# ViktorLiang/GW-Depth

Hardware: AMD Instinct MI355X
Metric: images/sec (train fwd+bwd) 480x640 bs=8/GPU (higher is better)
Workload: dtype bf16; 1 GPU; GW-Depth full model (res50 + DETR 6+6 + 4-scale ReferTransformer + decoder) fwd+17 losses+bwd+clip+AdamW, 480x640, bs=8/GPU, dropout 0.1; global_batch=8, parallelism=dp1, launch=hipgraph, graph_segments=1, grad_buckets=8

## Files before the change

gw_depth_amd/csrc/pyrtail.hip:

```cpp
#include "common.h"

namespace {

constexpr int PT_TH = 8, PT_TW = 8;
constexpr int PT_CH = 32;
constexpr int PT_MAXCHUNK = 10;
constexpr int PT_MAXR = 5, PT_MAXC = 5;
constexpr int PT_MAXPOS = PT_MAXR * PT_MAXC;
constexpr int PT_TAB = 128;
constexpr int PT_SPLIT = 4;

struct PyrBranches {
    void *p[GWD_PYR_MAX_BRANCHES];
    int h[GWD_PYR_MAX_BRANCHES], w[GWD_PYR_MAX_BRANCHES];
    int start[GWD_PYR_MAX_BRANCHES + 1];
    int n;
};

__device__ __forceinline__ float pt_scale(int in, int out) { return out > 1 ? (float)(in - 1) / (float)(out - 1) : 0.f; }

__device__ __forceinline__ float pt_weight(int o, int s, int in, float scale) {
    const float f = scale * o;
    const int i0 = (int)f, i1 = i0 + (i0 < in - 1);
    const float l = f - i0;
    return (i0 == s ? 1.f - l : 0.f) + (i1 == s ? l : 0.f);
}

template <typename T> struct Vec8;
template <> struct alignas(16) Vec8<__bf16> { __bf16 e[8]; };
template <> struct alignas(16) Vec8<float> { float e[8]; };

template <typename T> struct Raw8;
template <> struct Raw8<__bf16> { uint4 a; };
template <> struct Raw8<float> { uint4 a, b; };

template <typename T>
__device__ __forceinline__ void fma8(float (&acc)[8], float wgt, const Vec8<T> &v) {
#pragma unroll
    for (int e = 0; e < 8; ++e) acc[e] = fmaf(wgt, to_f32(v.e[e]), acc[e]);
}

template <typename T>
__global__ __launch_bounds__(256) void pyr_tail_fwd_kernel(const T *__restrict__ part, const PyrBranches br, const float *__restrict__ gamma,
                                                           const float *__restrict__ beta, T *__restrict__ z, T *__restrict__ y,
                                                           float *__restrict__ mean, float *__restrict__ rstd, int H, int W, int N, int gelu) {
    __shared__ Vec8<T> smz[PT_MAXPOS * 36];
    __shared__ Vec8<float> smh[PT_MAXR * 3 * PT_TW * 4];
    const int t = threadIdx.x, q = t & 3, pix = t >> 2;
    const int ntx = (W + PT_TW - 1) / PT_TW, nty = (H + PT_TH - 1) / PT_TH;
    const long vb = xcd_grouped_block(blockIdx.x, gridDim.x, 2 * ntx);
    const int px0 = (int)(vb % ntx) * PT_TW, py0 = (int)((vb / ntx) % nty) * PT_TH, b = (int)(vb / ((long)ntx * nty));
    const int pxl = pix & (PT_TW - 1);
    const int px = px0 + pxl, py = py0 + pix / PT_TW;
    const bool inside = px < W && py < H;
    const int nch = N / PT_CH;
    float acc[PT_MAXCHUNK][8];
#pragma unroll
    for (int j = 0; j < PT_MAXCHUNK; ++j)
#pragma unroll
        for (int e = 0; e < 8; ++e) acc[j][e] = 0.f;
    const int ya = max(py0 - 1, 0), yb = min(py0 + PT_TH, H - 1), xa = max(px0 - 1, 0), xb = min(px0 + PT_TW, W - 1);
    for (int k = 0; k < br.n; ++k) {
        const int h = br.h[k], w = br.w[k];
        const float sh = pt_scale(h, H), sw = pt_scale(w, W);
        const int rlo = (int)(sh * ya), rhi = min((int)(sh * yb) + 1, h - 1);
        const int clo = (int)(sw * xa), chi = min((int)(sw * xb) + 1, w - 1);
        const int nc = min(chi - clo + 1, PT_MAXC), nr = min(rhi - rlo + 1, PT_MAXR);
        const T *Zk = (const T *)br.p[k] + (size_t)b * h * w * 9 * N;
        static_assert(PT_MAXPOS * 36 <= 4 * 256, "four window places a thread");
        const int nitem = nr * nc * 36;
        auto place = [&](int u) {
            const int i = min(t + u * 256, nitem - 1);
            const int pos = i / 36, rem = i - pos * 36;
            return (((rlo + pos / nc) * w + clo + pos % nc) * 9 + (rem >> 2)) * N + (rem & 3) * 8;
        };
        const int zoff0 = place(0), zoff1 = place(1), zoff2 = place(2), zoff3 = place(3);
        typedef Raw8<T> R8;
        R8 pre0 = *(const R8 *)(Zk + zoff0), pre1 = *(const R8 *)(Zk + zoff1), pre2 = *(const R8 *)(Zk + zoff2), pre3 = *(const R8 *)(Zk + zoff3);
        R8 *smr = (R8 *)smz;
#pragma unroll
        for (int j = 0; j < PT_MAXCHUNK; ++j) {
            if (j < nch) {
                if (t < nitem) smr[t] = pre0;
                if (t + 256 < nitem) smr[t + 256] = pre1;
                if (t + 512 < nitem) smr[t + 512] = pre2;
                if (t + 768 < nitem) smr[t + 768] = pre3;
                __syncthreads();
                if (j + 1 < nch) {
                    const T *Zn = Zk + (j + 1) * PT_CH;
                    pre0 = *(const R8 *)(Zn + zoff0);
                    pre1 = *(const R8 *)(Zn + zoff1);
                    pre2 = *(const R8 *)(Zn + zoff2);
                    pre3 = *(const R8 *)(Zn + zoff3);
                }
                for (int i = t; i < nr * 3 * PT_TW * 4; i += 256) {
                    const int lane = i & 3, xl = (i >> 2) & (PT_TW - 1), rt = i / (PT_TW * 4);
                    const int rr = rt / 3, ty = rt - rr * 3;
                    Vec8<float> hv;
#pragma unroll
                    for (int e = 0; e < 8; ++e) hv.e[e] = 0.f;
#pragma unroll
                    for (int tx = 0; tx < 3; ++tx) {
                        const int xx = px0 + xl + tx - 1;
                        if (xx < 0 || xx >= W) continue;
                        const float fx = sw * xx;
                        const int c0 = (int)fx, c1 = c0 + (c0 < w - 1);
                        const float lx = fx - c0, hx = 1.f - lx;
                        const int tq = (ty * 3 + tx) * 4 + lane;
                        fma8<T>(hv.e, hx, smz[(rr * nc + min(c0 - clo, PT_MAXC - 1)) * 36 + tq]);
                        fma8<T>(hv.e, lx, smz[(rr * nc + min(c1 - clo, PT_MAXC - 1)) * 36 + tq]);
                    }
                    smh[i] = hv;
                }
                __syncthreads();
                if (inside) {
#pragma unroll
                    for (int ty = 0; ty < 3; ++ty) {
                        const int yy = py + ty - 1;
                        if (yy < 0 || yy >= H) continue;
                        const float fy = sh * yy;
                        const int r0 = (int)fy, r1 = r0 + (r0 < h - 1);
                        const float ly = fy - r0, hy = 1.f - ly;
                        fma8<float>(acc[j], hy, smh[((min(r0 - rlo, PT_MAXR - 1) * 3 + ty) * PT_TW + pxl) * 4 + q]);
                        fma8<float>(acc[j], ly, smh[((min(r1 - rlo, PT_MAXR - 1) * 3 + ty) * PT_TW + pxl) * 4 + q]);
                    }
                }
            }
        }
    }
    const size_t row = ((size_t)b * H + (inside ? py : 0)) * W + (inside ? px : 0);
    float s = 0.f;
#pragma unroll
    for (int j = 0; j < PT_MAXCHUNK; ++j) {
        if (j < nch && inside) {
            const size_t off = row * N + j * PT_CH + q * 8;
            const Vec8<T> pv = *(const Vec8<T> *)(part + off);
            Vec8<T> zv;
#pragma unroll
            for (int e = 0; e < 8; ++e) {
                zv.e[e] = from_f32<T>(acc[j][e] + to_f32(pv.e[e]));
                acc[j][e] = to_f32(zv.e[e]);
                s += acc[j][e];
            }
            if (z) *(Vec8<T> *)(z + off) = zv;
        }
    }
    s += __shfl_xor(s, 1, 64);
    s += __shfl_xor(s, 2, 64);
    const float mu = s / (float)N;
    float v2 = 0.f;
#pragma unroll
    for (int j = 0; j < PT_MAXCHUNK; ++j) {
        if (j < nch) {
#pragma unroll
            for (int e = 0; e < 8; ++e) {
                const float d = acc[j][e] - mu;
                v2 += d * d;
            }
        }
    }
    v2 += __shfl_xor(v2, 1, 64);
    v2 += __shfl_xor(v2, 2, 64);
    const float rs = rsqrtf(v2 / (float)N + 1e-5f);
    if (!inside) return;
    if (q == 0) {
        mean[row] = mu;
        rstd[row] = rs;
    }
#pragma unroll
    for (int j = 0; j < PT_MAXCHUNK; ++j) {
        if (j < nch) {
            const int ch = j * PT_CH + q * 8;
            Vec8<T> ov;
#pragma unroll
            for (int e = 0; e < 8; ++e) {
                float o = (acc[j][e] - mu) * rs * gamma[ch + e] + beta[ch + e];
                if (gelu) o = gelu_t<T>(o);
                ov.e[e] = from_f32<T>(o);
            }
            *(Vec8<T> *)(y + row * N + ch) = ov;
        }
    }
}

template <typename T>
__global__ __launch_bounds__(256) void pyr_tail_bwd_kernel(const T *__restrict__ gz, const PyrBranches br, int H, int W, int N) {
    __shared__ float sm[(PT_SPLIT - 1) * 9 * (PT_MAXCHUNK * 4) * 8];
    __shared__ float tabx[PT_TAB * 3], taby[PT_TAB * 3];
    const int lanes = N / 8, lane = threadIdx.x % lanes, grp = threadIdx.x / lanes;
    int k = 0;
    while (k + 1 < br.n && (int)blockIdx.x >= br.start[k + 1]) ++k;
    const int h = br.h[k], w = br.w[k];
    const int local = (int)xcd_grouped_block(blockIdx.x - br.start[k], br.start[k + 1] - br.start[k], 2 * w);
    const int c = local % w, r = (local / w) % h, b = local / (w * h);
    const float sh = pt_scale(h, H), sw = pt_scale(w, W);
    int ylo = 0, yhi = H - 1, xlo = 0, xhi = W - 1;
    if (sh > 0.f) {
        ylo = max(0, (int)floorf((r - 1) / sh) - 2);
        yhi = min(H - 1, (int)ceilf((r + 1) / sh) + 2);
    }
    if (sw > 0.f) {
        xlo = max(0, (int)floorf((c - 1) / sw) - 2);
        xhi = min(W - 1, (int)ceilf((c + 1) / sw) + 2);
    }
    auto wx_of = [&](int xx, int tx) {
        const int sx = xx + tx - 1;
        return (sx >= 0 && sx < W) ? pt_weight(sx, c, w, sw) : 0.f;
    };
    while (xlo < xhi && wx_of(xlo, 0) == 0.f && wx_of(xlo, 1) == 0.f && wx_of(xlo, 2) == 0.f) ++xlo;
    while (xhi > xlo && wx_of(xhi, 0) == 0.f && wx_of(xhi, 1) == 0.f && wx_of(xhi, 2) == 0.f) --xhi;
    auto wy_of = [&](int yy, int ty) {
        const int sy = yy + ty - 1;
        return (sy >= 0 && sy < H) ? pt_weight(sy, r, h, sh) : 0.f;
    };
    const bool tab = xhi - xlo < PT_TAB && yhi - ylo < PT_TAB;
    if (tab) {
        for (int i = threadIdx.x; i < (xhi - xlo + 1) * 3; i += blockDim.x) tabx[i] = wx_of(xlo + i / 3, i % 3);
        for (int i = threadIdx.x; i < (yhi - ylo + 1) * 3; i += blockDim.x) taby[i] = wy_of(ylo + i / 3, i % 3);
        __syncthreads();
    }
    float acc[9][8];
#pragma unroll
    for (int i = 0; i < 9; ++i)
#pragma unroll
        for (int e = 0; e < 8; ++e) acc[i][e] = 0.f;
    const T *gb = gz + (size_t)b * H * W * N + lane * 8;
    for (int yy = ylo + grp; yy <= yhi; yy += PT_SPLIT) {
        float wy[3];
#pragma unroll
        for (int ty = 0; ty < 3; ++ty) wy[ty] = tab ? taby[(yy - ylo) * 3 + ty] : wy_of(yy, ty);
        if (wy[0] == 0.f && wy[1] == 0.f && wy[2] == 0.f) continue;
        float rowsum[3][8];
#pragma unroll
        for (int i = 0; i < 3; ++i)
#pragma unroll
            for (int e = 0; e < 8; ++e) rowsum[i][e] = 0.f;
#pragma unroll 4
        for (int xx = xlo; xx <= xhi; ++xx) {
            float wx[3];
#pragma unroll
            for (int tx = 0; tx < 3; ++tx) wx[tx] = tab ? tabx[(xx - xlo) * 3 + tx] : wx_of(xx, tx);
            const Vec8<T> v = *(const Vec8<T> *)(gb + ((size_t)yy * W + xx) * N);
#pragma unroll
            for (int tx = 0; tx < 3; ++tx) fma8<T>(rowsum[tx], wx[tx], v);
        }
#pragma unroll
        for (int ty = 0; ty < 3; ++ty)
#pragma unroll
            for (int tx = 0; tx < 3; ++tx)
#pragma unroll
                for (int e = 0; e < 8; ++e) acc[ty * 3 + tx][e] = fmaf(wy[ty], rowsum[tx][e], acc[ty * 3 + tx][e]);
    }
    if (grp > 0) {
#pragma unroll
        for (int i = 0; i < 9; ++i)
#pragma unroll
            for (int e = 0; e < 8; ++e) sm[(((grp - 1) * 9 + i) * lanes + lane) * 8 + e] = acc[i][e];
    }
    __syncthreads();
    if (grp == 0) {
        T *G = (T *)br.p[k] + ((size_t)(b * h + r) * w + c) * 9 * N + lane * 8;
#pragma unroll
        for (int i = 0; i < 9; ++i) {
            Vec8<T> ov;
#pragma unroll
            for (int e = 0; e < 8; ++e) {
                float v = acc[i][e];
#pragma unroll
                for (int g = 0; g < PT_SPLIT - 1; ++g) v += sm[((g * 9 + i) * lanes + lane) * 8 + e];
                ov.e[e] = from_f32<T>(v);
            }
            *(Vec8<T> *)(G + (size_t)i * N) = ov;
        }
    }
}

struct PyrFold {
    const float *lo[GWD_PYR_MAX_BRANCHES];
};
__global__ __launch_bounds__(256) void pyr_tail_fold_kernel(const float *__restrict__ d_hi, const PyrFold lo, float *__restrict__ dw, int N,
                                                            int C2, int nbr, int nlow, int64_t total) {
    const int64_t i = (int64_t)blockIdx.x * 256 + threadIdx.x;
    if (i >= total) return;
    const int Cw = (1 + nbr) * C2, Chi = (1 + nbr - nlow) * C2;
    const int ch = (int)(i % Cw);
    const int64_t nt = i / Cw;
    const int tap = (int)(nt % 9), n = (int)(nt / 9);
    const int g = ch / C2, ci = ch - g * C2;
    float v;
    if (g == 0) v = d_hi[nt * Chi + ci];
    else if (g <= nlow) v = lo.lo[g - 1][((size_t)tap * N + n) * C2 + ci];
    else v = d_hi[nt * Chi + (g - nlow) * C2 + ci];
    dw[i] += v;
}

int check_branches(const int32_t *hk, const int32_t *wk, int nb, int H, int W) {
    for (int k = 0; k < nb; ++k) {
        if (hk[k] <= 0 || wk[k] <= 0 || hk[k] > H || wk[k] > W) return -1;
    }
    return 0;
}

}

extern "C" int gwd_pyr_tail_forward(const void *part, const void *const *Z, const int32_t *hk, const int32_t *wk, int32_t nb,
                                    const float *gamma, const float *beta, void *z, void *y, float *mean, float *rstd, int32_t B,
                                    int32_t H, int32_t W, int32_t N, int32_t gelu, int32_t dtype, void *stream) {
    if (!part || !Z || !hk || !wk || !gamma || !beta || !y || !mean || !rstd || B <= 0 || H <= 0 || W <= 0 || N <= 0) return -1;
    if (nb < 1 || nb > GWD_PYR_MAX_BRANCHES || check_branches(hk, wk, nb, H, W)) return -1;
    if (dtype != GWD_BF16 && dtype != GWD_F32) return -2;
    if (N % PT_CH || N > PT_CH * PT_MAXCHUNK) return -4;
    PyrBranches br = {};
    br.n = nb;
    for (int k = 0; k < nb; ++k) {
        if (!Z[k]) return -1;
        const double sh = H > 1 ? (double)(hk[k] - 1) / (H - 1) : 0.0, sw = W > 1 ? (double)(wk[k] - 1) / (W - 1) : 0.0;
        int nr = (int)(sh * (PT_TH + 1) * (1.0 + 1e-6)) + 3, nc = (int)(sw * (PT_TW + 1) * (1.0 + 1e-6)) + 3;
        nr = nr < hk[k] ? nr : hk[k];
        nc = nc < wk[k] ? nc : wk[k];
        if (nr > PT_MAXR || nc > PT_MAXC) return -4;
        br.p[k] = const_cast<void *>(Z[k]);
        br.h[k] = hk[k];
        br.w[k] = wk[k];
    }
    const int64_t nblk = (int64_t)B * ((W + PT_TW - 1) / PT_TW) * ((H + PT_TH - 1) / PT_TH);
    if (nblk >= (1LL << 31)) return -7;
    const int grid = (int)nblk;
    if (dtype == GWD_BF16)
        pyr_tail_fwd_kernel<__bf16><<<grid, 256, 0, (hipStream_t)stream>>>((const __bf16 *)part, br, gamma, beta, (__bf16 *)z, (__bf16 *)y, mean,
                                                                           rstd, H, W, N, gelu);
    else
        pyr_tail_fwd_kernel<float><<<grid, 256, 0, (hipStream_t)stream>>>((const float *)part, br, gamma, beta, (float *)z, (float *)y, mean, rstd,
                                                                          H, W, N, gelu);
    GWD_CHECK_LAUNCH();
    return 0;
}

extern "C" int gwd_pyr_tail_backward(const void *gz, void *const *G, const int32_t *hk, const int32_t *wk, int32_t nb, int32_t B, int32_t H,
                                     int32_t W, int32_t N, int32_t dtype, void *stream) {
    if (!gz || !G || !hk || !wk || B <= 0 || H <= 0 || W <= 0 || N <= 0) return -1;
    if (nb < 1 || nb > GWD_PYR_MAX_BRANCHES || check_branches(hk, wk, nb, H, W)) return -1;
    if (dtype != GWD_BF16 && dtype != GWD_F32) return -2;
    if (N % 8 || N > PT_CH * PT_MAXCHUNK) return -4;
    PyrBranches br = {};
    br.n = nb;
    int64_t blocks = 0;
    for (int k = 0; k < nb; ++k) {
        if (!G[k]) return -1;
        br.p[k] = G[k];
        br.h[k] = hk[k];
        br.w[k] = wk[k];
        br.start[k] = (int)blocks;
        blocks += (int64_t)B * hk[k] * wk[k];
        if (blocks >= (1LL << 31)) return -7;
    }
    br.start[nb] = (int)blocks;
    const int threads = N / 8 * PT_SPLIT;
    if (dtype == GWD_BF16) pyr_tail_bwd_kernel<__bf16><<<(int)blocks, threads, 0, (hipStream_t)stream>>>((const __bf16 *)gz, br, H, W, N);
    else pyr_tail_bwd_kernel<float><<<(int)blocks, threads, 0, (hipStream_t)stream>>>((const float *)gz, br, H, W, N);
    GWD_CHECK_LAUNCH();
    return 0;
}

extern "C" int gwd_pyr_tail_fold_wgrad(const float *d_hi, const float *const *d_low, int32_t nlow, float *dw, int32_t N, int32_t C2,
                                       int32_t nbr, void *stream) {
    if (!d_hi || !d_low || !dw || N <= 0 || C2 <= 0 || nbr < 1 || nbr > GWD_PYR_MAX_BRANCHES || nlow < 1 || nlow > nbr) return -1;
    PyrFold lo = {};
    for (int k = 0; k < nlow; ++k) {
        if (!d_low[k]) return -1;
        lo.lo[k] = d_low[k];
    }
    const int64_t total = (int64_t)N * 9 * (1 + nbr) * C2;
    if ((total + 255) / 256 >= (1LL << 31)) return -7;
    pyr_tail_fold_kernel<<<(int)((total + 255) / 256), 256, 0, (hipStream_t)stream>>>(d_hi, lo, dw, N, C2, nbr, nlow, total);
    GWD_CHECK_LAUNCH();
    return 0;
}
```

Baseline: 264.5 images/s.

## Double-buffer pyramid tail forward, widen to 8 lanes per pixel, precompute interp offsets

The pyramid-tail forward kernel goes from 256 to 512 threads, with 8 lanes per pixel each handling 4 channels instead of 4 lanes handling 8. Window tiles and horizontal sums are double-buffered in shared memory, so the next chunk's global loads and shared stores overlap compute and one barrier per chunk is dropped. Bilinear indices and weights are hoisted out of the chunk loop into per-thread registers, and gamma and beta are loaded as float4. In the backward kernel the table/no-table branch is hoisted out of the inner loop and pointer increments replace index arithmetic. The costs are doubled shared memory and a larger block, which may lower occupancy.

```diff
diff --git a/gw_depth_amd/csrc/pyrtail.hip b/gw_depth_amd/csrc/pyrtail.hip
--- a/gw_depth_amd/csrc/pyrtail.hip
+++ b/gw_depth_amd/csrc/pyrtail.hip
@@ -3,6 +3,8 @@
 namespace {
 
 constexpr int PT_TH = 8, PT_TW = 8;
+constexpr int PT_LANES = 8;
+constexpr int PT_FTHREADS = PT_TH * PT_TW * PT_LANES;
 constexpr int PT_CH = 32;
 constexpr int PT_MAXCHUNK = 10;
 constexpr int PT_MAXR = 5, PT_MAXC = 5;
@@ -19,12 +21,24 @@
 
 __device__ __forceinline__ float pt_scale(int in, int out) { return out > 1 ? (float)(in - 1) / (float)(out - 1) : 0.f; }
 
+__device__ __forceinline__ void pt_coord(int o, float scale, int &i0, float &l) {
+#pragma clang fp contract(off)
+    const float f = scale * o;
+    i0 = (int)f;
+    l = f - i0;
+}
+
 __device__ __forceinline__ float pt_weight(int o, int s, int in, float scale) {
-    const float f = scale * o;
-    const int i0 = (int)f, i1 = i0 + (i0 < in - 1);
-    const float l = f - i0;
+    int i0;
+    float l;
+    pt_coord(o, scale, i0, l);
+    const int i1 = i0 + (i0 < in - 1);
     return (i0 == s ? 1.f - l : 0.f) + (i1 == s ? l : 0.f);
 }
+
+template <typename T> struct Vec4;
+template <> struct alignas(8) Vec4<__bf16> { __bf16 e[4]; };
+template <> struct alignas(16) Vec4<float> { float e[4]; };
 
 template <typename T> struct Vec8;
 template <> struct alignas(16) Vec8<__bf16> { __bf16 e[8]; };
@@ -35,18 +49,25 @@
 template <> struct Raw8<float> { uint4 a, b; };
 
 template <typename T>
+__device__ __forceinline__ void fma4(float (&acc)[4], float wgt, const Vec4<T> &v) {
+#pragma unroll
+    for (int e = 0; e < 4; ++e) acc[e] = fmaf(wgt, to_f32(v.e[e]), acc[e]);
+}
+
+template <typename T>
 __device__ __forceinline__ void fma8(float (&acc)[8], float wgt, const Vec8<T> &v) {
 #pragma unroll
     for (int e = 0; e < 8; ++e) acc[e] = fmaf(wgt, to_f32(v.e[e]), acc[e]);
 }
 
 template <typename T>
-__global__ __launch_bounds__(256) void pyr_tail_fwd_kernel(const T *__restrict__ part, const PyrBranches br, const float *__restrict__ gamma,
-                                                           const float *__restrict__ beta, T *__restrict__ z, T *__restrict__ y,
-                                                           float *__restrict__ mean, float *__restrict__ rstd, int H, int W, int N, int gelu) {
-    __shared__ Vec8<T> smz[PT_MAXPOS * 36];
-    __shared__ Vec8<float> smh[PT_MAXR * 3 * PT_TW * 4];
-    const int t = threadIdx.x, q = t & 3, pix = t >> 2;
+__global__ __launch_bounds__(PT_FTHREADS) __attribute__((amdgpu_waves_per_eu(2, 4))) void pyr_tail_fwd_kernel(
+    const T *__restrict__ part, const PyrBranches br, const float *__restrict__ gamma, const float *__restrict__ beta, T *__restrict__ z,
+    T *__restrict__ y, float *__restrict__ mean, float *__restrict__ rstd, int H, int W, int N, int gelu) {
+    typedef Raw8<T> R8;
+    __shared__ R8 smz[2][PT_MAXPOS * 36];
+    __shared__ Vec4<float> smh[2][PT_MAXR * 3 * PT_TW * PT_LANES];
+    const int t = threadIdx.x, q = t & (PT_LANES - 1), pix = t / PT_LANES;
     const int ntx = (W + PT_TW - 1) / PT_TW, nty = (H + PT_TH - 1) / PT_TH;
     const long vb = xcd_grouped_block(blockIdx.x, gridDim.x, 2 * ntx);
     const int px0 = (int)(vb % ntx) * PT_TW, py0 = (int)((vb / ntx) % nty) * PT_TH, b = (int)(vb / ((long)ntx * nty));
@@ -54,12 +75,13 @@
     const int px = px0 + pxl, py = py0 + pix / PT_TW;
     const bool inside = px < W && py < H;
     const int nch = N / PT_CH;
-    float acc[PT_MAXCHUNK][8];
+    float acc[PT_MAXCHUNK][4];
 #pragma unroll
     for (int j = 0; j < PT_MAXCHUNK; ++j)
 #pragma unroll
-        for (int e = 0; e < 8; ++e) acc[j][e] = 0.f;
+        for (int e = 0; e < 4; ++e) acc[j][e] = 0.f;
     const int ya = max(py0 - 1, 0), yb = min(py0 + PT_TH, H - 1), xa = max(px0 - 1, 0), xb = min(px0 + PT_TW, W - 1);
+    const Vec4<T> *smz4 = (const Vec4<T> *)smz;
     for (int k = 0; k < br.n; ++k) {
         const int h = br.h[k], w = br.w[k];
         const float sh = pt_scale(h, H), sw = pt_scale(w, W);
@@ -67,63 +89,95 @@
         const int clo = (int)(sw * xa), chi = min((int)(sw * xb) + 1, w - 1);
         const int nc = min(chi - clo + 1, PT_MAXC), nr = min(rhi - rlo + 1, PT_MAXR);
         const T *Zk = (const T *)br.p[k] + (size_t)b * h * w * 9 * N;
-        static_assert(PT_MAXPOS * 36 <= 4 * 256, "four window places a thread");
+        static_assert(PT_MAXPOS * 36 <= 2 * PT_FTHREADS, "two window places a thread");
         const int nitem = nr * nc * 36;
         auto place = [&](int u) {
-            const int i = min(t + u * 256, nitem - 1);
+            const int i = min(t + u * PT_FTHREADS, nitem - 1);
             const int pos = i / 36, rem = i - pos * 36;
             return (((rlo + pos / nc) * w + clo + pos % nc) * 9 + (rem >> 2)) * N + (rem & 3) * 8;
         };
-        const int zoff0 = place(0), zoff1 = place(1), zoff2 = place(2), zoff3 = place(3);
-        typedef Raw8<T> R8;
-        R8 pre0 = *(const R8 *)(Zk + zoff0), pre1 = *(const R8 *)(Zk + zoff1), pre2 = *(const R8 *)(Zk + zoff2), pre3 = *(const R8 *)(Zk + zoff3);
-        R8 *smr = (R8 *)smz;
+        const int zoff0 = place(0), zoff1 = place(1);
+        R8 pre0 = *(const R8 *)(Zk + zoff0), pre1 = *(const R8 *)(Zk + zoff1);
+        static_assert(PT_MAXR * 3 <= 2 * (PT_FTHREADS / 64), "two horizontal items a thread");
+        int hoff0[3], hoff1[3];
+        float hx[3], lx[3];
+#pragma unroll
+        for (int tx = 0; tx < 3; ++tx) {
+            const int xx = px0 + pxl + tx - 1;
+            const bool ok = xx >= 0 && xx < W;
+            int c0;
+            float l;
+            pt_coord(ok ? xx : 0, sw, c0, l);
+            const int c1 = c0 + (c0 < w - 1);
+            hx[tx] = ok ? 1.f - l : 0.f;
+            lx[tx] = ok ? l : 0.f;
+            hoff0[tx] = min(max(c0 - clo, 0), nc - 1) * 72 + tx * 8;
+            hoff1[tx] = min(max(c1 - clo, 0), nc - 1) * 72 + tx * 8;
+        }
+        const int rt0 = t >> 6, rt1 = rt0 + PT_FTHREADS / 64;
+        const int hbase0 = (rt0 / 3) * nc * 72 + (rt0 % 3) * 24 + q, hbase1 = (rt1 / 3) * nc * 72 + (rt1 % 3) * 24 + q;
+        const bool hdo0 = rt0 < nr * 3, hdo1 = rt1 < nr * 3;
+        int voff0[3], voff1[3];
+        float hy[3], ly[3];
+#pragma unroll
+        for (int ty = 0; ty < 3; ++ty) {
+            const int yy = py + ty - 1;
+            const bool ok = inside && yy >= 0 && yy < H;
+            int r0;
+            float l;
+            pt_coord(ok ? yy : 0, sh, r0, l);
+            const int r1 = r0 + (r0 < h - 1);
+            hy[ty] = ok ? 1.f - l : 0.f;
+            ly[ty] = ok ? l : 0.f;
+            voff0[ty] = ((min(max(r0 - rlo, 0), nr - 1) * 3 + ty) * PT_TW + pxl) * PT_LANES + q;
+            voff1[ty] = ((min(max(r1 - rlo, 0), nr - 1) * 3 + ty) * PT_TW + pxl) * PT_LANES + q;
+        }
+        if (t < nitem) smz[0][t] = pre0;
+        if (t + PT_FTHREADS < nitem) smz[0][t + PT_FTHREADS] = pre1;
+        if (nch > 1) {
+            pre0 = *(const R8 *)(Zk + PT_CH + zoff0);
+            pre1 = *(const R8 *)(Zk + PT_CH + zoff1);
+        }
+        __syncthreads();
 #pragma unroll
         for (int j = 0; j < PT_MAXCHUNK; ++j) {
             if (j < nch) {
-                if (t < nitem) smr[t] = pre0;
-                if (t + 256 < nitem) smr[t + 256] = pre1;
-                if (t + 512 < nitem) smr[t + 512] = pre2;
-                if (t + 768 < nitem) smr[t + 768] = pre3;
-                __syncthreads();
+                constexpr int PIECES = PT_MAXPOS * 72, SUMS = PT_MAXR * 3 * PT_TW * PT_LANES;
+                const Vec4<T> *wz = smz4 + (j & 1) * PIECES;
+                Vec4<float> *wh = smh[j & 1];
                 if (j + 1 < nch) {
-                    const T *Zn = Zk + (j + 1) * PT_CH;
-                    pre0 = *(const R8 *)(Zn + zoff0);
-                    pre1 = *(const R8 *)(Zn + zoff1);
-                    pre2 = *(const R8 *)(Zn + zoff2);
-                    pre3 = *(const R8 *)(Zn + zoff3);
+                    if (t < nitem) smz[(j + 1) & 1][t] = pre0;
+                    if (t + PT_FTHREADS < nitem) smz[(j + 1) & 1][t + PT_FTHREADS] = pre1;
+                    if (j + 2 < nch) {
+                        const T *Zn = Zk + (j + 2) * PT_CH;
+                        pre0 = *(const R8 *)(Zn + zoff0);
+                        pre1 = *(const R8 *)(Zn + zoff1);
+                    }
                 }
-                for (int i = t; i < nr * 3 * PT_TW * 4; i += 256) {
-                    const int lane = i & 3, xl = (i >> 2) & (PT_TW - 1), rt = i / (PT_TW * 4);
-                    const int rr = rt / 3, ty = rt - rr * 3;
-                    Vec8<float> hv;
-#pragma unroll
-                    for (int e = 0; e < 8; ++e) hv.e[e] = 0.f;
+                if (hdo0) {
+                    Vec4<float> hv = {{0.f, 0.f, 0.f, 0.f}};
 #pragma unroll
                     for (int tx = 0; tx < 3; ++tx) {
-                        const int xx = px0 + xl + tx - 1;
-                        if (xx < 0 || xx >= W) continue;
-                        const float fx = sw * xx;
-                        const int c0 = (int)fx, c1 = c0 + (c0 < w - 1);
-                        const float lx = fx - c0, hx = 1.f - lx;
-                        const int tq = (ty * 3 + tx) * 4 + lane;
-                        fma8<T>(hv.e, hx, smz[(rr * nc + min(c0 - clo, PT_MAXC - 1)) * 36 + tq]);
-                        fma8<T>(hv.e, lx, smz[(rr * nc + min(c1 - clo, PT_MAXC - 1)) * 36 + tq]);
+                        fma4<T>(hv.e, hx[tx], wz[hbase0 + hoff0[tx]]);
+                        fma4<T>(hv.e, lx[tx], wz[hbase0 + hoff1[tx]]);
                     }
-                    smh[i] = hv;
+                    wh[t] = hv;
+                }
+                if (hdo1) {
+                    Vec4<float> hv = {{0.f, 0.f, 0.f, 0.f}};
+#pragma unroll
+                    for (int tx = 0; tx < 3; ++tx) {
+                        fma4<T>(hv.e, hx[tx], wz[hbase1 + hoff0[tx]]);
+                        fma4<T>(hv.e, lx[tx], wz[hbase1 + hoff1[tx]]);
+                    }
+                    wh[t + PT_FTHREADS] = hv;
                 }
                 __syncthreads();
-                if (inside) {
-#pragma unroll
-                    for (int ty = 0; ty < 3; ++ty) {
-                        const int yy = py + ty - 1;
-                        if (yy < 0 || yy >= H) continue;
-                        const float fy = sh * yy;
-                        const int r0 = (int)fy, r1 = r0 + (r0 < h - 1);
-                        const float ly = fy - r0, hy = 1.f - ly;
-                        fma8<float>(acc[j], hy, smh[((min(r0 - rlo, PT_MAXR - 1) * 3 + ty) * PT_TW + pxl) * 4 + q]);
-                        fma8<float>(acc[j], ly, smh[((min(r1 - rlo, PT_MAXR - 1) * 3 + ty) * PT_TW + pxl) * 4 + q]);
-                    }
+                static_assert(SUMS >= 15 * 64, "smh holds every horizontal item");
+#pragma unroll
+                for (int ty = 0; ty < 3; ++ty) {
+                    fma4<float>(acc[j], hy[ty], wh[voff0[ty]]);
+                    fma4<float>(acc[j], ly[ty], wh[voff1[ty]]);
                 }
             }
         }
@@ -133,34 +187,34 @@
 #pragma unroll
     for (int j = 0; j < PT_MAXCHUNK; ++j) {
         if (j < nch && inside) {
-            const size_t off = row * N + j * PT_CH + q * 8;
-            const Vec8<T> pv = *(const Vec8<T> *)(part + off);
-            Vec8<T> zv;
-#pragma unroll
-            for (int e = 0; e < 8; ++e) {
+            const size_t off = row * N + j * PT_CH + q * 4;
+            const Vec4<T> pv = *(const Vec4<T> *)(part + off);
+            Vec4<T> zv;
+#pragma unroll
+            for (int e = 0; e < 4; ++e) {
                 zv.e[e] = from_f32<T>(acc[j][e] + to_f32(pv.e[e]));
                 acc[j][e] = to_f32(zv.e[e]);
                 s += acc[j][e];
             }
-            if (z) *(Vec8<T> *)(z + off) = zv;
-        }
-    }
-    s += __shfl_xor(s, 1, 64);
-    s += __shfl_xor(s, 2, 64);
+            if (z) *(Vec4<T> *)(z + off) = zv;
+        }
+    }
+#pragma unroll
+    for (int o = 1; o < PT_LANES; o <<= 1) s += __shfl_xor(s, o, 64);
     const float mu = s / (float)N;
     float v2 = 0.f;
 #pragma unroll
     for (int j = 0; j < PT_MAXCHUNK; ++j) {
         if (j < nch) {
 #pragma unroll
-            for (int e = 0; e < 8; ++e) {
+            for (int e = 0; e < 4; ++e) {
                 const float d = acc[j][e] - mu;
                 v2 += d * d;
             }
         }
     }
-    v2 += __shfl_xor(v2, 1, 64);
-    v2 += __shfl_xor(v2, 2, 64);
+#pragma unroll
+    for (int o = 1; o < PT_LANES; o <<= 1) v2 += __shfl_xor(v2, o, 64);
     const float rs = rsqrtf(v2 / (float)N + 1e-5f);
     if (!inside) return;
     if (q == 0) {
@@ -170,15 +224,17 @@
 #pragma unroll
     for (int j = 0; j < PT_MAXCHUNK; ++j) {
         if (j < nch) {
-            const int ch = j * PT_CH + q * 8;
-            Vec8<T> ov;
-#pragma unroll
-            for (int e = 0; e < 8; ++e) {
-                float o = (acc[j][e] - mu) * rs * gamma[ch + e] + beta[ch + e];
+            const int ch = j * PT_CH + q * 4;
+            const float4 gm = *(const float4 *)(gamma + ch), bt = *(const float4 *)(beta + ch);
+            const float gv[4] = {gm.x, gm.y, gm.z, gm.w}, bv[4] = {bt.x, bt.y, bt.z, bt.w};
+            Vec4<T> ov;
+#pragma unroll
+            for (int e = 0; e < 4; ++e) {
+                float o = (acc[j][e] - mu) * rs * gv[e] + bv[e];
                 if (gelu) o = gelu_t<T>(o);
                 ov.e[e] = from_f32<T>(o);
             }
-            *(Vec8<T> *)(y + row * N + ch) = ov;
+            *(Vec4<T> *)(y + row * N + ch) = ov;
         }
     }
 }
@@ -227,22 +283,34 @@
     const T *gb = gz + (size_t)b * H * W * N + lane * 8;
     for (int yy = ylo + grp; yy <= yhi; yy += PT_SPLIT) {
         float wy[3];
-#pragma unroll
-        for (int ty = 0; ty < 3; ++ty) wy[ty] = tab ? taby[(yy - ylo) * 3 + ty] : wy_of(yy, ty);
+        if (tab) {
+#pragma unroll
+            for (int ty = 0; ty < 3; ++ty) wy[ty] = taby[(yy - ylo) * 3 + ty];
+        } else {
+#pragma unroll
+            for (int ty = 0; ty < 3; ++ty) wy[ty] = wy_of(yy, ty);
+        }
         if (wy[0] == 0.f && wy[1] == 0.f && wy[2] == 0.f) continue;
         float rowsum[3][8];
 #pragma unroll
         for (int i = 0; i < 3; ++i)
 #pragma unroll
             for (int e = 0; e < 8; ++e) rowsum[i][e] = 0.f;
+        const T *gp = gb + ((size_t)yy * W + xlo) * N;
+        if (tab) {
+            const float *wp = tabx;
 #pragma unroll 4
-        for (int xx = xlo; xx <= xhi; ++xx) {
-            float wx[3];
-#pragma unroll
-            for (int tx = 0; tx < 3; ++tx) wx[tx] = tab ? tabx[(xx - xlo) * 3 + tx] : wx_of(xx, tx);
-            const Vec8<T> v = *(const Vec8<T> *)(gb + ((size_t)yy * W + xx) * N);
-#pragma unroll
-            for (int tx = 0; tx < 3; ++tx) fma8<T>(rowsum[tx], wx[tx], v);
+            for (int xx = xlo; xx <= xhi; ++xx, gp += N, wp += 3) {
+                const Vec8<T> v = *(const Vec8<T> *)gp;
+#pragma unroll
+                for (int tx = 0; tx < 3; ++tx) fma8<T>(rowsum[tx], wp[tx], v);
+            }
+        } else {
+            for (int xx = xlo; xx <= xhi; ++xx, gp += N) {
+                const Vec8<T> v = *(const Vec8<T> *)gp;
+#pragma unroll
+                for (int tx = 0; tx < 3; ++tx) fma8<T>(rowsum[tx], wx_of(xx, tx), v);
+            }
         }
 #pragma unroll
         for (int ty = 0; ty < 3; ++ty)
@@ -327,10 +395,10 @@
     if (nblk >= (1LL << 31)) return -7;
     const int grid = (int)nblk;
     if (dtype == GWD_BF16)
-        pyr_tail_fwd_kernel<__bf16><<<grid, 256, 0, (hipStream_t)stream>>>((const __bf16 *)part, br, gamma, beta, (__bf16 *)z, (__bf16 *)y, mean,
+        pyr_tail_fwd_kernel<__bf16><<<grid, PT_FTHREADS, 0, (hipStream_t)stream>>>((const __bf16 *)part, br, gamma, beta, (__bf16 *)z, (__bf16 *)y, mean,
                                                                            rstd, H, W, N, gelu);
     else
-        pyr_tail_fwd_kernel<float><<<grid, 256, 0, (hipStream_t)stream>>>((const float *)part, br, gamma, beta, (float *)z, (float *)y, mean, rstd,
+        pyr_tail_fwd_kernel<float><<<grid, PT_FTHREADS, 0, (hipStream_t)stream>>>((const float *)part, br, gamma, beta, (float *)z, (float *)y, mean, rstd,
                                                                           H, W, N, gelu);
     GWD_CHECK_LAUNCH();
     return 0;
```

Measured after the change: 266.2 images/s, median of 6. Within noise of the previous version (+0.6%).
